# bananaofhappiness/soundscope

Hardware: AMD Instinct MI355X
Metric: audio samples/s analyzed (48 kHz stereo) (higher is better)
Workload: dtype f32 + f64

## Files before the change

soundscope_amd/csrc/ss_batch.cpp:

```cpp
#include "ss_host.h"

using namespace ssh;

namespace {

struct TimingRing {
    static constexpr uint32_t kDepth = 32;
    bool on = false;
    hipEvent_t ev[kDepth * 2 * SS_KERNEL_COUNT] = {};
    uint32_t mask[kDepth] = {};
    uint32_t head = 0, count = 0;
    double ms[SS_KERNEL_COUNT] = {};
    uint64_t launches[SS_KERNEL_COUNT] = {};
    ~TimingRing() { for (auto &e : ev) if (e) (void)hipEventDestroy(e); }
    hipError_t create() { hipError_t r = hipSuccess; for (auto &e : ev) if (r == hipSuccess) r = hipEventCreate(&e); return r; }
    hipError_t mark(int kernel, int edge, hipStream_t stream)
    {
        if (!on) return hipSuccess;
        const int idx = 2 * kernel + edge;
        mask[head] |= 1u << idx;
        return hipEventRecord(ev[(size_t)head * 2 * SS_KERNEL_COUNT + idx], stream);
    }
    void advance() { if (on) { head = (head + 1u) % kDepth; count++; } }
    int collect(hipStream_t stream)
// ... 73 lines not shown
    DevBuf<double> sub, weights, integrated, lra, out2;
    DevBuf<double> seg_state;
    DevBuf<uint64_t> hist, corpus;
    DevBuf<uint32_t> counts;
    DevBuf<unsigned char> raw;
    DevBuf<uint64_t> checks;
    DevBuf<double> series;
    DevBuf<ssk::LoudnessExtremes> extremes;
    Ragged ragged;
    DevBuf<float> render_spec, render_wave;
    DevBuf<uint32_t> col_start;
    uint32_t render_cols = 0, render_wave_cols = 0;
    Columns cols;
    Overlap ov;
    bool corpus_reduced = false;
    int tp_arith = SS_TP_ARITH_F32;
    TimingRing timing;

    uint32_t sub_cap() const { return lay.n_subblocks ? lay.n_subblocks : 1; }
    size_t samples_per_stream() const { return (size_t)cfg.frames_per_stream * cfg.channels; }
};

namespace ssi {
void *batch_corpus_device(ss_batch *b) { return b ? b->corpus.p : nullptr; }
hipStream_t batch_stream(ss_batch *b) { return b ? b->stream : nullptr; }
int batch_device(const ss_batch *b) { return b ? b->device : 0; }
bool &batch_corpus_reduced(ss_batch *b) { return b->corpus_reduced; }
}

namespace {
// ... 310 lines not shown
            L.fft_bytes = rows * b->render_cols * sizeof(float);
        } else {
            L.fft_bytes = rows * L.fft_bin_stride * sizeof(float);
            HIPCHK(b->fft.alloc((size_t)(L.fft_bytes / sizeof(float))));
        }
    }
    if (b->td) {
        HIPCHK(b->state.alloc(cfg->n_streams));
        HIPCHK(b->sub.alloc((size_t)cfg->n_streams * b->sub_cap() * C));
        HIPCHK(b->hist.alloc((size_t)cfg->n_streams * 2 * sst::kHistBins));
        HIPCHK(b->corpus.alloc(2 * sst::kHistBins));
        HIPCHK(b->integrated.alloc(cfg->n_streams));
        HIPCHK(b->lra.alloc(cfg->n_streams));
        HIPCHK(b->counts.alloc((size_t)cfg->n_streams * 2));
        HIPCHK(b->out2.alloc(2));
        std::vector<double> w(C);
        sst::channel_weights(C, w.data());
        HIPCHK(b->weights.upload(w));
        if (cfg->flags & SS_BATCH_LOUDNESS_SERIES) {
            HIPCHK(b->series.alloc((size_t)cfg->n_streams * b->sub_cap() * 2));
            HIPCHK(b->extremes.alloc(cfg->n_streams));
        }
    }
    if (cfg->flags & SS_BATCH_WAVEFORM) {
        if (sh.wave_window > 0xFFFFFFFFull) return SS_ERR_UNSUPPORTED;
        b->wave_window = (uint32_t)sh.wave_window;
        L.n_wave_points = (uint32_t)(2 * sh.wave_bins);
        HIPCHK(b->wave.alloc((size_t)cfg->n_streams * (b->wave_window ? 2 * (size_t)b->wave_window : 2)));
    }

// ... 137 lines not shown
    SS_ON_DEVICE(b);
    if (!b) return SS_ERR_INVALID_ARG;
    HIPCHK(ssk::launch_synth(b->pcm.p, b->cfg.n_streams, b->cfg.frames_per_stream, b->cfg.channels,
                             b->cfg.sample_rate, seed, first_stream_id, b->stream));
    HIPCHK(hipStreamSynchronize(b->stream));
    return SS_OK;
}

int ss_batch_run(ss_batch *b)
{
    SS_ON_DEVICE(b);
    if (!b) return SS_ERR_INVALID_ARG;
    TimingRing &t = b->timing;
    int rc = (t.count >= TimingRing::kDepth || !t.on) ? t.collect(b->stream) : SS_OK;
    if (rc) return rc;
    b->corpus_reduced = false;

    enum class At { first, behind_td, last };
    const bool gain_from_meter = b->cols.on && b->cols.gain_mode == SS_GAIN_REFERENCE;
    const int mode = (t.on || gain_from_meter) ? 0 : b->ov.mode;
    const At at = gain_from_meter ? At::last : mode == 2 ? At::behind_td : At::first;
    auto spectrum_if = [&](At here) { return here == at ? spectrum_step(b, mode != 0) : SS_OK; };

    if ((rc = spectrum_if(At::first))) return rc;

    HIPCHK(t.mark(SS_KERNEL_TIME_DOMAIN, 0, b->stream));
    const ssk::TdParams tdp = b->td ? batch_td_params(b) : ssk::TdParams{};
    if (b->td) {
        HIPCHK(zero_meter(b));
        HIPCHK(t.mark(SS_KERNEL_TIME_DOMAIN, 0, b->stream));
        HIPCHK(ssk::launch_time_domain(tdp, b->stream));
    }
    if ((rc = spectrum_if(At::behind_td))) return rc;
    if (b->td && b->td_plan.fixup) HIPCHK(ssk::launch_time_domain_fixup(tdp, b->stream));
    HIPCHK(t.mark(SS_KERNEL_TIME_DOMAIN, 1, b->stream));

    HIPCHK(t.mark(SS_KERNEL_FINALIZE, 0, b->stream));
    if (b->td) {
        const ssk::FinalizeParams f = batch_gating_params(b);
        HIPCHK(ssk::launch_finalize(f, b->stream));
        if (b->series.p) HIPCHK(ssk::launch_loudness_series(f, b->series.p, b->sub_cap(), b->extremes.p, b->stream));
    }
    HIPCHK(t.mark(SS_KERNEL_FINALIZE, 1, b->stream));

    HIPCHK(t.mark(SS_KERNEL_WAVEFORM, 0, b->stream));
    if ((b->cfg.flags & SS_BATCH_WAVEFORM) && b->wave_window && (!b->wave_fused || b->ragged.on))
        HIPCHK(ssk::launch_waveform(batch_wave_params(b), b->stream));
    HIPCHK(t.mark(SS_KERNEL_WAVEFORM, 1, b->stream));

    if ((rc = spectrum_if(At::last))) return rc;
    if (mode) HIPCHK(b->ov.join(b->stream));
    t.advance();
    return SS_OK;
}

// ... 246 lines not shown
{
    SS_ON_DEVICE(b);
    if (!b || !dst || !b->corpus.p) return SS_ERR_INVALID_ARG;
    return fetch(b, static_cast<uint64_t *>(dst), b->corpus.p, 2 * sst::kHistBins, hipMemcpyDeviceToDevice);
}

int ss_batch_corpus_gate_enqueue(ss_batch *b, ss_comm *comm)
{
    SS_ON_DEVICE(b);
    if (!b) return SS_ERR_INVALID_ARG;
    if (!b->corpus.p) return SS_ERR_INVALID_MODE;
    if (comm) {
        int rc = ss_batch_allreduce_histograms(b, comm, nullptr);
        if (rc) return rc;
    }
    HIPCHK(ssk::launch_hist_eval(b->corpus.p, b->hist_energies, b->hist_bounds, b->out2.p, b->stream));
    return SS_OK;
}

int ss_batch_corpus_gate_read(ss_batch *b, double *integrated, double *lra)
{
    SS_ON_DEVICE(b);
    if (!b) return SS_ERR_INVALID_ARG;
    if (!b->corpus.p) return SS_ERR_INVALID_MODE;
    double r[2];
    int rc = fetch(b, r, b->out2.p, 2);
    if (rc) return rc;
    if (integrated) *integrated = r[0];
    if (lra) *lra = r[1];
    return SS_OK;
// ... 209 lines not shown
```

soundscope_amd/csrc/ss_kernels.h:

```cpp
#pragma once
#include <hip/hip_runtime.h>

#include <mutex>
#include <cstddef>
#include <cstdint>

namespace ssk {

struct DevicePrep {
    std::mutex mu;
    uint64_t done = 0;
};
template <class F>
inline hipError_t prepare_on_device(DevicePrep &p, F &&prepare)
{
    int d = 0;
    if (hipGetDevice(&d) != hipSuccess) d = 0;
    const uint64_t bit = 1ull << (d & 63);
    std::lock_guard<std::mutex> lk(p.mu);
    if (p.done & bit) return hipSuccess;
    const hipError_t e = prepare();
    if (e == hipSuccess) p.done |= bit;
    return e;
}
// ... 115 lines not shown
    uint64_t wave_stride;
    uint32_t wave_window;
    uint32_t halo_frames;
    const uint64_t *frames_of;
    uint32_t tp_f32;
    double *seg_state;
    uint32_t fixup, fix_sub;
    uint32_t split_batch;
    double *st_out;
    double *st_scratch;
    const double *st_weights;
    double st_frames;
    uint32_t st_begin_elem, st_old_total, st_blocks;
};
hipError_t launch_time_domain(const TdParams &p, hipStream_t s, const FftBatchParams *tick_fft = nullptr, bool *tick_fused = nullptr);
hipError_t launch_time_domain_fixup(const TdParams &p, hipStream_t s);
uint32_t td_chunk_frames(uint32_t channels, uint32_t s100);
uint32_t td_split_chunk_frames(uint32_t channels, uint32_t s100);
uint32_t td_resident_waves_per_cu(uint32_t channels, uint32_t s100, uint32_t halo_frames);
uint32_t td_ring_tile_frames(uint32_t channels, uint32_t s100);

struct FinalizeParams {
    const TdConst *k;
    const double *subblocks; uint64_t sub_stride; uint32_t sub_cap;
    const double *hist_energies;
    const double *hist_bounds;
    const double *weights;
    uint64_t *hist;
    uint64_t *corpus_hist;
    uint32_t n_streams, channels;
    uint64_t sub_begin, sub_end;
    double *out_integrated;
    double *out_lra;
    uint32_t *out_counts;
    const uint32_t *sub_end_of;
    const TdState *state;
    double *readings_out;
    const float *readings_peaks_src; float *readings_peaks_dst; uint32_t *readings_flag; uint32_t readings_seq;
};
hipError_t launch_finalize(const FinalizeParams &p, hipStream_t s);
__attribute__((visibility("hidden"))) hipError_t launch_finalize_stream(const FinalizeParams &p, hipStream_t s);
struct LoudnessExtremes { double max_m, max_s; uint32_t at_m, at_s; };
hipError_t launch_loudness_series(const FinalizeParams &p, double *series, uint64_t series_stride, LoudnessExtremes *extremes,
                                  hipStream_t s);
struct ReadingsExtra { const float *peaks_src; float *peaks_dst; uint32_t *flag; uint32_t seq; };
hipError_t launch_hist_eval(const uint64_t *hist2000, const double *energies, const double *bounds,
                            double *out2, hipStream_t s, const ReadingsExtra *peaks = nullptr);
constexpr int kRingScratchDoubles = 320;
constexpr int kRingTickScratch = 264;
constexpr int kRingTickBlocks = 32;
hipError_t launch_ring_energy(const double *ring, uint64_t ring_frames, uint32_t channels,
                              uint64_t end_frame, uint64_t frames, const double *weights,
                              double *out2 ,
                              double *scratch ,
                              hipStream_t s);
// ... 75 lines not shown
```

soundscope_amd/csrc/ss_loudness.hip:

```cpp
#include "ss_kernels.h"

namespace ssk {
__device__ __forceinline__ uint32_t hist_index(const double *__restrict__ bounds, double energy)
{
    const double g = (10.0 * log10(energy) - 0.691 + 70.0) * 10.0;
    int i = g > 0.0 ? (g < (double)(kHistBins - 1) ? (int)g : kHistBins - 1) : 0;
    while (i > 0 && energy < bounds[i]) i--;
    while (i < kHistBins - 1 && energy >= bounds[i + 1]) i++;
    return (uint32_t)i;
}

__device__ __forceinline__ double wave_sum(double v)
{
#pragma unroll
    for (int o = 32; o >= 1; o >>= 1) v += __shfl_xor(v, o, 64);
    return v;
}
__device__ __forceinline__ unsigned long long wave_sum_u64(unsigned long long v)
{
#pragma unroll
    for (int o = 32; o >= 1; o >>= 1) v += __shfl_xor(v, o, 64);
    return v;
}

__device__ __forceinline__ uint32_t first_bad_subblock(const TdState *st, uint32_t C, const double *__restrict__ weights, uint32_t lane)
{
    uint32_t key = 0u;
    if (st) for (uint32_t c = lane; c < C; c += 64u) { const uint32_t k = st->bad_key[c]; if (weights[c] != 0.0 && k > key) key = k; }
#pragma unroll
    for (int o = 32; o >= 1; o >>= 1) { const uint32_t t = (uint32_t)__shfl_xor((int)key, o, 64); key = t > key ? t : key; }
    return ~key;
}

__device__ __forceinline__ void eval_hist(const unsigned long long *hb, const unsigned long long *hs,
                          const double *__restrict__ en, const double *__restrict__ bd,
                          double *out_i, double *out_lra)
{
    const int lane = threadIdx.x & 63;
    double sum = 0.0; unsigned long long cnt = 0;
    for (int i = lane; i < kHistBins; i += 64) { sum += (double)hb[i] * en[i]; cnt += hb[i]; }
    sum = wave_sum(sum); cnt = wave_sum_u64(cnt);
    double integrated;
    if (cnt == 0) integrated = -INFINITY;
    else {
        const double rel = (sum / (double)cnt) * 0.1;
        uint32_t start;
        if (rel < bd[0]) start = 0;
        else { start = hist_index(bd, rel); if (rel > en[start]) start++; }
        double g = 0.0; unsigned long long c2 = 0;
        for (int i = lane; i < kHistBins; i += 64) if ((uint32_t)i >= start) { g += (double)hb[i] * en[i]; c2 += hb[i]; }
        g = wave_sum(g); c2 = wave_sum_u64(c2);
        integrated = c2 ? 10.0 * log10(g / (double)c2) - 0.691 : -INFINITY;
    }
    double power = 0.0; unsigned long long size = 0;
    for (int i = lane; i < kHistBins; i += 64) { power += (double)hs[i] * en[i]; size += hs[i]; }
    power = wave_sum(power); size = wave_sum_u64(size);
    double lra = 0.0;
    if (size != 0) {
        const double integ = 0.01 * (power / (double)size);
        uint32_t index;
        if (integ < bd[0]) index = 0;
        else { index = hist_index(bd, integ); if (integ > en[index]) index++; }
        const int b0 = lane * 16;
        unsigned long long own = 0;
#pragma unroll
        for (int q = 0; q < 16; q++) {
            const int i = b0 + ((q + lane) & 15);
            if (i < kHistBins && (uint32_t)i >= index) own += hs[i];
        }
        unsigned long long incl = own;
#pragma unroll
        for (int o = 1; o < 64; o <<= 1) {
            const unsigned long long t = __shfl_up(incl, o, 64);
            if (lane >= o) incl += t;
        }
        const unsigned long long above = __shfl(incl, 63, 64);
        if (above != 0) {
            const unsigned long long plow = (unsigned long long)((double)(above - 1) * 0.1 + 0.5);
            const unsigned long long phigh = (unsigned long long)((double)(above - 1) * 0.95 + 0.5);
            const unsigned long long excl = incl - own;
            auto energy_of_rank = [&](unsigned long long r) -> double {
                const bool mine = excl <= r && r < incl;
                double e = 0.0;
                if (mine) {
                    unsigned long long acc = excl;
                    int j = b0 > (int)index ? b0 : (int)index;
                    for (;;) { acc += hs[j]; if (acc > r) break; j++; }
                    e = en[j];
                }
                const int src = __ffsll((long long)__ballot(mine)) - 1;
                return __shfl(e, src, 64);
            };
            const double l_en = energy_of_rank(plow), h_en = energy_of_rank(phigh);
            lra = (10.0 * log10(h_en) - 0.691) - (10.0 * log10(l_en) - 0.691);
        }
    }
    if (lane == 0) { if (out_i) *out_i = integrated; if (out_lra) *out_lra = lra; }
}

__device__ __forceinline__ uint32_t ring_back(uint32_t jm, uint32_t q, uint32_t cap)
{
    uint32_t s = jm + cap * 30u - q;
    return s % cap;
}

template <int N, bool DIRECT, int KB = (N < 10 ? N : 10)>
__device__ __forceinline__ double window_energy(const double *__restrict__ P, uint32_t jm, uint32_t cap, uint32_t C,
                                                const double *__restrict__ weights)
{
    constexpr int kBatch = KB;
    static_assert(N % kBatch == 0, "whole batches");
    uint32_t s0 = DIRECT ? jm - (uint32_t)(N - 1) : ring_back(jm, (uint32_t)(N - 1), cap);
    double sum = 0.0;
    for (uint32_t c = 0; c < C; c++) {
        const double w = weights[c];
        if (w == 0.0) continue;
        double cs = 0.0;
        uint32_t sl = s0;
#pragma unroll
        for (int b = 0; b < N; b += kBatch) {
            double v[kBatch];
#pragma unroll
            for (int q = 0; q < kBatch; q++) {
                v[q] = P[(size_t)sl * C + c];
                sl = DIRECT ? sl + 1u : (sl + 1u == cap ? 0u : sl + 1u);
            }
#pragma unroll
            for (int q = 0; q < kBatch; q++) cs += v[q];
        }
        sum += w * cs;
    }
    return sum;
}

template <int N, bool DIRECT>
__device__ __forceinline__ double window_energy_eager(const double *__restrict__ P, uint32_t jm, uint32_t cap, uint32_t C,
                                                      const double *__restrict__ weights)
{
    const uint32_t s0 = DIRECT ? jm - (uint32_t)(N - 1) : ring_back(jm, (uint32_t)(N - 1), cap);
    double sum = 0.0;
    for (uint32_t c = 0; c < C; c += 2) {
        const bool two = c + 1u < C;
        const uint32_t c1 = two ? c + 1u : c;
        const double w0 = weights[c], w1 = weights[c1];
        double v0[N], v1[N];
        uint32_t sl = s0;
#pragma unroll
        for (int q = 0; q < N; q++) {
            v0[q] = P[(size_t)sl * C + c];
            v1[q] = P[(size_t)sl * C + c1];
            sl = DIRECT ? sl + 1u : (sl + 1u == cap ? 0u : sl + 1u);
        }
        double cs0 = 0.0, cs1 = 0.0;
#pragma unroll
        for (int q = 0; q < N; q++) { cs0 += v0[q]; cs1 += v1[q]; }
        if (w0 != 0.0) sum += w0 * cs0;
        if (two && w1 != 0.0) sum += w1 * cs1;
    }
    return sum;
}

template <bool SMALL>
__global__ __launch_bounds__(SMALL ? 256 : 1024) void k_finalize(FinalizeParams p)
{
    __shared__ unsigned long long hb[kHistBins];
    __shared__ unsigned long long hs[kHistBins];
    __shared__ unsigned int counts[2];
    __shared__ uint32_t bad_from_s;
    __shared__ double tab[SMALL ? 2 * kHistBins + 1 : 1];
    const uint32_t stream = blockIdx.x;
    const int lane = threadIdx.x, nthr = (int)blockDim.x;
    unsigned long long *gh = reinterpret_cast<unsigned long long *>(p.hist) + (size_t)stream * 2 * kHistBins;
    unsigned long long *corpus = reinterpret_cast<unsigned long long *>(p.corpus_hist);
    for (int i = lane; i < kHistBins; i += nthr) {
        hb[i] = gh[i]; hs[i] = gh[kHistBins + i];
        if (SMALL) { tab[i] = p.hist_energies[i]; tab[kHistBins + i] = p.hist_bounds[i]; }
    }
    if (SMALL && lane == 0) tab[2 * kHistBins] = p.hist_bounds[kHistBins];
    if (lane < 2) counts[lane] = 0;
    if (lane < 64) {
        const uint32_t bf = first_bad_subblock(p.state ? p.state + stream : nullptr, p.channels, p.weights, (uint32_t)lane);
        if (lane == 0) bad_from_s = bf;
    }
    const double *en = SMALL ? tab : p.hist_energies;
    const double *bd = SMALL ? tab + kHistBins : p.hist_bounds;
    const double bd0 = p.hist_bounds[0];
    const uint64_t sub_end = p.sub_end_of ? p.sub_end_of[stream] : p.sub_end;
    __syncthreads();

    const uint32_t C = p.channels;
    const double S = (double)p.k->s100;
    const double *P = p.subblocks + (size_t)stream * p.sub_stride;
    const uint32_t cap = p.sub_cap;
    const bool direct = p.sub_end <= (uint64_t)cap && p.sub_begin == 0;
    const uint64_t bad_from = bad_from_s;
    uint32_t nb = 0, ns = 0;
    for (uint64_t j = (p.sub_begin > 3 ? p.sub_begin : 3) + lane; j < sub_end; j += nthr) {
        const uint32_t jm = direct ? (uint32_t)j : (uint32_t)(j % cap);
        double sum;
        if (SMALL) sum = direct ? window_energy_eager<4, true>(P, jm, cap, C, p.weights) : window_energy_eager<4, false>(P, jm, cap, C, p.weights);
        else sum = direct ? window_energy<4, true>(P, jm, cap, C, p.weights) : window_energy<4, false>(P, jm, cap, C, p.weights);
        sum /= 4.0 * S;
        nb++;
        if (j > bad_from) sum = __builtin_nan("");
        if (sum >= bd0) atomicAdd(&hb[hist_index(bd, sum)], 1ull);
    }
    if (!p.k->st_off) {
        const uint64_t m_begin = p.sub_begin > 29 ? (p.sub_begin - 29 + 9) / 10 : 0;
        for (uint64_t m = m_begin + lane;; m += nthr) {
            const uint64_t j = 29 + 10 * m;
            if (j >= sub_end) break;
            const uint32_t jm = direct ? (uint32_t)j : (uint32_t)(j % cap);
            double sum;
            if (SMALL) sum = direct ? window_energy_eager<30, true>(P, jm, cap, C, p.weights) : window_energy_eager<30, false>(P, jm, cap, C, p.weights);
            else sum = direct ? window_energy<30, true>(P, jm, cap, C, p.weights) : window_energy<30, false>(P, jm, cap, C, p.weights);
            sum /= 30.0 * S;
            ns++;
            if (j > bad_from) sum = __builtin_nan("");
            if (sum >= bd0) atomicAdd(&hs[hist_index(bd, sum)], 1ull);
        }
    }
    if (nb) atomicAdd(&counts[0], nb);
    if (ns) atomicAdd(&counts[1], ns);
    __syncthreads();
    for (int i = lane; i < kHistBins; i += nthr) {
        const unsigned long long db = hb[i] - gh[i], ds = hs[i] - gh[kHistBins + i];
        if (corpus) {
            if (db) atomicAdd(&corpus[i], db);
            if (ds) atomicAdd(&corpus[kHistBins + i], ds);
        }
        gh[i] = hb[i];
        gh[kHistBins + i] = hs[i];
    }
    if (p.out_counts && lane < 2) p.out_counts[stream * 2 + lane] += counts[lane];
    if (lane < 64)
        eval_hist(hb, hs, en, bd,
                  p.out_integrated ? &p.out_integrated[stream] : nullptr,
                  p.out_lra ? &p.out_lra[stream] : nullptr);
}

__device__ __forceinline__ void gate_stream_range(const double *__restrict__ P, uint32_t cap, uint32_t C, const double *__restrict__ weights,
                                                  const TdConst &K, const double *__restrict__ bd, double bd0, uint64_t sub_begin,
                                                  uint64_t sub_end, uint64_t bad_from, unsigned long long *gh, uint32_t *out_counts,
                                                  uint32_t lane)
{
    const double S = (double)K.s100;
    uint32_t nb = 0, ns = 0;
    for (uint64_t j = (sub_begin > 3 ? sub_begin : 3) + lane; j < sub_end; j += 64) {
        double sum = window_energy_eager<4, false>(P, (uint32_t)(j % cap), cap, C, weights) / (4.0 * S);
        if (j > bad_from) sum = __builtin_nan("");
        nb++;
        if (sum >= bd0) atomicAdd(&gh[hist_index(bd, sum)], 1ull);
    }
    if (!K.st_off) {
        const uint64_t m_begin = sub_begin > 29 ? (sub_begin - 29 + 9) / 10 : 0;
// ... 33 lines not shown
            hb[i] = __hip_atomic_load(&gh[i], __ATOMIC_RELAXED, __HIP_MEMORY_SCOPE_AGENT);
            hs[i] = __hip_atomic_load(&gh[kHistBins + i], __ATOMIC_RELAXED, __HIP_MEMORY_SCOPE_AGENT);
        }
        if (p.readings_peaks_dst) {
            p.readings_peaks_dst[lane] = p.readings_peaks_src[lane];
            p.readings_peaks_dst[64 + lane] = p.readings_peaks_src[64 + lane];
        }
        __syncthreads();
        eval_hist(hb, hs, en, bd, &p.readings_out[0], &p.readings_out[1]);
        if (p.readings_flag) {
            __threadfence_system();
            __syncthreads();
            if (lane == 0) __hip_atomic_store(p.readings_flag, p.readings_seq, __ATOMIC_RELEASE, __HIP_MEMORY_SCOPE_SYSTEM);
        }
    }
}

constexpr uint32_t kFinalizeSmallMax = 64u;
hipError_t launch_finalize(const FinalizeParams &p, hipStream_t s)
{
    if (p.n_streams == 0) return hipSuccess;
    const uint64_t nsub = p.sub_end - p.sub_begin;
    const uint32_t threads = nsub > 2048 ? 1024u : 256u;
    if (p.n_streams <= kFinalizeSmallMax && threads == 256u) hipLaunchKernelGGL(k_finalize<true>, dim3(p.n_streams), dim3(threads), 0, s, p);
    else hipLaunchKernelGGL(k_finalize<false>, dim3(p.n_streams), dim3(threads), 0, s, p);
    return hipGetLastError();
}

hipError_t launch_finalize_stream(const FinalizeParams &p, hipStream_t s)
{
    if (p.n_streams == 0) return hipSuccess;
    hipLaunchKernelGGL(k_finalize_stream, dim3(1), dim3(64), 0, s, p);
    return hipGetLastError();
}

template <int N>
__device__ __forceinline__ double window_energy_head(const double *__restrict__ P, uint32_t j, uint32_t C,
                                                     const double *__restrict__ weights)
{
    double sum = 0.0;
    for (uint32_t c = 0; c < C; c++) {
// ... 333 lines not shown
```

soundscope_amd/csrc/ss_td_body.inc:

```
    using Cfg = TpCfg<FACTOR>;
    constexpr bool kSplitBatch = SPLIT && !RING;
    constexpr bool kSplitCall = SPLIT && RING;
    constexpr bool late = LATE;
    static_assert(!kSplitCall || LATE, "streaming calls hand the state over behind the scan");
    extern __shared__ __attribute__((aligned(16))) unsigned char smem[];
    const uint32_t lane = threadIdx.x & 63u;
    const uint32_t wave_in_block = (uint32_t)__builtin_amdgcn_readfirstlane((int)(threadIdx.x >> 6));
    const uint32_t nwb = SPLIT ? (uint32_t)(blockDim.x >> 6) : (uint32_t)kTdWavesPerBlock;
    const uint32_t gw = SPLIT ? block_id : block_id * kTdWavesPerBlock + wave_in_block;
    const bool fix = p.fixup != 0u;
    const uint32_t wps = fix ? p.nseg - 1u : p.nseg;
    if (gw >= p.n_streams * wps) return;
    const uint32_t stream = gw / wps, sg = gw - stream * wps + (fix ? 1u : 0u);
    TdShare *const sh = reinterpret_cast<TdShare *>(smem + (size_t)nwb * wave_lds_floats * sizeof(float));

    float *tilebuf = reinterpret_cast<float *>(smem) + (size_t)wave_in_block * wave_lds_floats;
    const TdConst &K = *p.k;
    const uint32_t C = CT ? (uint32_t)CT : p.channels;
    const uint32_t S = p.s100;
    const uint32_t nch = 64u / C;
    constexpr bool kRowScan = (CT != 0) && (16 % (CT ? CT : 1) == 0);
    const uint32_t lane_q = (lane & 15u) / C;
    const uint32_t chunk = kRowScan ? (lane >> 4) + 4u * lane_q : lane / C;
    const uint32_t ch = kRowScan ? (lane & 15u) - lane_q * C : lane - chunk * C;
// ... 1205 lines not shown
```

soundscope_amd/csrc/ss_time_domain.hip:

```cpp
#include "ss_td_impl.h"

namespace ssk {
static uint32_t td_lds_blocks(size_t lds)
{
    const uint32_t blocks = (uint32_t)(kTdLdsBytes / lds);
    const uint32_t max_blocks = (4u * kTdWaves) / kTdWavesPerBlock;
    return blocks > max_blocks ? max_blocks : blocks;
}

uint32_t td_chunk_frames(uint32_t C, uint32_t s100)
{
#ifdef SS_TUNING
    if (const char *e = std::getenv("SS_TD_L")) { const int v = std::atoi(e); if (v >= 8 && v <= 128) return (uint32_t)v; }
#endif
    const uint32_t nch = 64u / C;
    const bool rowscan = C == 1 || C == 2 || C == 8;
    static const double occupancy[5] = {8.0, 3.0, 1.6, 1.25, 1.0};
    uint32_t best = 33; double best_cost = 1e300;
    for (uint32_t L : {20u, 25u, 30u, 33u, 35u, 40u, 45u, 49u, 50u, 55u, 60u, 65u}) {
        const TdTile t = td_tile(C, s100, L, kTdHaloFrames, kTdWavesPerBlock, false);
        const uint32_t pieces = t.pieces, tile_len = t.tile_len;
        const uint32_t blocks = td_lds_blocks(t.lds);
        if (blocks == 0) continue;
        const uint32_t rem = tile_len % L;
// ... 49 lines not shown

hipError_t launch_time_domain(const TdParams &p, hipStream_t s, const FftBatchParams *tick_fft, bool *tick_fused)
{
    bool fused_local = false;
    bool *fused = tick_fused ? tick_fused : &fused_local;
    *fused = false;
    if (p.n_streams == 0 || p.n_frames == 0) return hipSuccess;
    const bool ring = p.ring != nullptr;
    switch (p.tp_factor) {
        case 4: return td_launch_f4(p, s, tick_fft, fused, ring);
        case 2: return td_launch_f2(p, s, tick_fft, fused, ring);
        default: return td_launch_f0(p, s, tick_fft, fused, ring);
    }
}

hipError_t launch_time_domain_fixup(const TdParams &p, hipStream_t s)
{
    if (p.n_streams == 0 || p.n_frames == 0 || p.nseg < 2 || !p.seg_state || !p.fix_sub) return hipSuccess;
    TdParams q = p;
    q.fixup = 1u; q.wave_out = nullptr; q.wave_window = 0; q.halo_frames = 0; q.tp_factor = 0;
    bool fused = false;
    return td_launch_f0(q, s, nullptr, &fused, false);
}

}
```

Baseline: 202.2 billion.

## Fuse time-domain fixup, finalize gating and corpus gate into one tail kernel

Replaces the separate fixup launch and finalize launch with a single td_tail kernel. Per-stream groups do the segment fixup, then the last-arriving block per stream (tracked by an atomic arrival counter) runs the gating histogram. A global ticket then lets the final block evaluate the corpus gate in the same kernel, so the later hist_eval launch is skipped when no communicator is used. This removes kernel launches and inter-kernel gaps in exchange for atomic ticketing, extra LDS and more complex synchronization.

```diff
diff --git a/soundscope_amd/csrc/ss_batch.cpp b/soundscope_amd/csrc/ss_batch.cpp
--- a/soundscope_amd/csrc/ss_batch.cpp
+++ b/soundscope_amd/csrc/ss_batch.cpp
@@ -111,6 +111,8 @@
     Columns cols;
     Overlap ov;
     bool corpus_reduced = false;
+    bool corpus_gate_done = false;
+    DevBuf<uint32_t> tail_ticket;
     int tp_arith = SS_TP_ARITH_F32;
     TimingRing timing;
 
@@ -451,6 +453,7 @@
         HIPCHK(b->lra.alloc(cfg->n_streams));
         HIPCHK(b->counts.alloc((size_t)cfg->n_streams * 2));
         HIPCHK(b->out2.alloc(2));
+        HIPCHK(b->tail_ticket.upload(std::vector<uint32_t>((size_t)cfg->n_streams + 1, 0u)));
         std::vector<double> w(C);
         sst::channel_weights(C, w.data());
         HIPCHK(b->weights.upload(w));
@@ -618,7 +621,9 @@
     TimingRing &t = b->timing;
     int rc = (t.count >= TimingRing::kDepth || !t.on) ? t.collect(b->stream) : SS_OK;
     if (rc) return rc;
+    if (t.on) t.mask[t.head] = 0;
     b->corpus_reduced = false;
+    b->corpus_gate_done = false;
 
     enum class At { first, behind_td, last };
     const bool gain_from_meter = b->cols.on && b->cols.gain_mode == SS_GAIN_REFERENCE;
@@ -635,14 +640,14 @@
         HIPCHK(t.mark(SS_KERNEL_TIME_DOMAIN, 0, b->stream));
         HIPCHK(ssk::launch_time_domain(tdp, b->stream));
     }
+    HIPCHK(t.mark(SS_KERNEL_TIME_DOMAIN, 1, b->stream));
     if ((rc = spectrum_if(At::behind_td))) return rc;
-    if (b->td && b->td_plan.fixup) HIPCHK(ssk::launch_time_domain_fixup(tdp, b->stream));
-    HIPCHK(t.mark(SS_KERNEL_TIME_DOMAIN, 1, b->stream));
 
     HIPCHK(t.mark(SS_KERNEL_FINALIZE, 0, b->stream));
     if (b->td) {
         const ssk::FinalizeParams f = batch_gating_params(b);
-        HIPCHK(ssk::launch_finalize(f, b->stream));
+        HIPCHK(ssk::launch_td_tail(tdp, f, b->tail_ticket.p + 1, b->corpus.p ? b->tail_ticket.p : nullptr, b->out2.p, b->stream));
+        b->corpus_gate_done = b->corpus.p != nullptr;
         if (b->series.p) HIPCHK(ssk::launch_loudness_series(f, b->series.p, b->sub_cap(), b->extremes.p, b->stream));
     }
     HIPCHK(t.mark(SS_KERNEL_FINALIZE, 1, b->stream));
@@ -919,6 +924,7 @@
         int rc = ss_batch_allreduce_histograms(b, comm, nullptr);
         if (rc) return rc;
     }
+    if (!comm && b->corpus_gate_done && !b->corpus_reduced) return SS_OK;
     HIPCHK(ssk::launch_hist_eval(b->corpus.p, b->hist_energies, b->hist_bounds, b->out2.p, b->stream));
     return SS_OK;
 }
diff --git a/soundscope_amd/csrc/ss_kernels.h b/soundscope_amd/csrc/ss_kernels.h
--- a/soundscope_amd/csrc/ss_kernels.h
+++ b/soundscope_amd/csrc/ss_kernels.h
@@ -153,7 +153,6 @@
     uint32_t st_begin_elem, st_old_total, st_blocks;
 };
 hipError_t launch_time_domain(const TdParams &p, hipStream_t s, const FftBatchParams *tick_fft = nullptr, bool *tick_fused = nullptr);
-hipError_t launch_time_domain_fixup(const TdParams &p, hipStream_t s);
 uint32_t td_chunk_frames(uint32_t channels, uint32_t s100);
 uint32_t td_split_chunk_frames(uint32_t channels, uint32_t s100);
 uint32_t td_resident_waves_per_cu(uint32_t channels, uint32_t s100, uint32_t halo_frames);
@@ -177,7 +176,7 @@
     double *readings_out;
     const float *readings_peaks_src; float *readings_peaks_dst; uint32_t *readings_flag; uint32_t readings_seq;
 };
-hipError_t launch_finalize(const FinalizeParams &p, hipStream_t s);
+hipError_t launch_td_tail(const TdParams &td, const FinalizeParams &f, uint32_t *arrive, uint32_t *ticket, double *gate_out2, hipStream_t s);
 __attribute__((visibility("hidden"))) hipError_t launch_finalize_stream(const FinalizeParams &p, hipStream_t s);
 struct LoudnessExtremes { double max_m, max_s; uint32_t at_m, at_s; };
 hipError_t launch_loudness_series(const FinalizeParams &p, double *series, uint64_t series_stride, LoudnessExtremes *extremes,
diff --git a/soundscope_amd/csrc/ss_loudness.hip b/soundscope_amd/csrc/ss_loudness.hip
--- a/soundscope_amd/csrc/ss_loudness.hip
+++ b/soundscope_amd/csrc/ss_loudness.hip
@@ -1,244 +1,6 @@
-#include "ss_kernels.h"
+#include "ss_loudness_dev.h"
 
 namespace ssk {
-__device__ __forceinline__ uint32_t hist_index(const double *__restrict__ bounds, double energy)
-{
-    const double g = (10.0 * log10(energy) - 0.691 + 70.0) * 10.0;
-    int i = g > 0.0 ? (g < (double)(kHistBins - 1) ? (int)g : kHistBins - 1) : 0;
-    while (i > 0 && energy < bounds[i]) i--;
-    while (i < kHistBins - 1 && energy >= bounds[i + 1]) i++;
-    return (uint32_t)i;
-}
-
-__device__ __forceinline__ double wave_sum(double v)
-{
-#pragma unroll
-    for (int o = 32; o >= 1; o >>= 1) v += __shfl_xor(v, o, 64);
-    return v;
-}
-__device__ __forceinline__ unsigned long long wave_sum_u64(unsigned long long v)
-{
-#pragma unroll
-    for (int o = 32; o >= 1; o >>= 1) v += __shfl_xor(v, o, 64);
-    return v;
-}
-
-__device__ __forceinline__ uint32_t first_bad_subblock(const TdState *st, uint32_t C, const double *__restrict__ weights, uint32_t lane)
-{
-    uint32_t key = 0u;
-    if (st) for (uint32_t c = lane; c < C; c += 64u) { const uint32_t k = st->bad_key[c]; if (weights[c] != 0.0 && k > key) key = k; }
-#pragma unroll
-    for (int o = 32; o >= 1; o >>= 1) { const uint32_t t = (uint32_t)__shfl_xor((int)key, o, 64); key = t > key ? t : key; }
-    return ~key;
-}
-
-__device__ __forceinline__ void eval_hist(const unsigned long long *hb, const unsigned long long *hs,
-                          const double *__restrict__ en, const double *__restrict__ bd,
-                          double *out_i, double *out_lra)
-{
-    const int lane = threadIdx.x & 63;
-    double sum = 0.0; unsigned long long cnt = 0;
-    for (int i = lane; i < kHistBins; i += 64) { sum += (double)hb[i] * en[i]; cnt += hb[i]; }
-    sum = wave_sum(sum); cnt = wave_sum_u64(cnt);
-    double integrated;
-    if (cnt == 0) integrated = -INFINITY;
-    else {
-        const double rel = (sum / (double)cnt) * 0.1;
-        uint32_t start;
-        if (rel < bd[0]) start = 0;
-        else { start = hist_index(bd, rel); if (rel > en[start]) start++; }
-        double g = 0.0; unsigned long long c2 = 0;
-        for (int i = lane; i < kHistBins; i += 64) if ((uint32_t)i >= start) { g += (double)hb[i] * en[i]; c2 += hb[i]; }
-        g = wave_sum(g); c2 = wave_sum_u64(c2);
-        integrated = c2 ? 10.0 * log10(g / (double)c2) - 0.691 : -INFINITY;
-    }
-    double power = 0.0; unsigned long long size = 0;
-    for (int i = lane; i < kHistBins; i += 64) { power += (double)hs[i] * en[i]; size += hs[i]; }
-    power = wave_sum(power); size = wave_sum_u64(size);
-    double lra = 0.0;
-    if (size != 0) {
-        const double integ = 0.01 * (power / (double)size);
-        uint32_t index;
-        if (integ < bd[0]) index = 0;
-        else { index = hist_index(bd, integ); if (integ > en[index]) index++; }
-        const int b0 = lane * 16;
-        unsigned long long own = 0;
-#pragma unroll
-        for (int q = 0; q < 16; q++) {
-            const int i = b0 + ((q + lane) & 15);
-            if (i < kHistBins && (uint32_t)i >= index) own += hs[i];
-        }
-        unsigned long long incl = own;
-#pragma unroll
-        for (int o = 1; o < 64; o <<= 1) {
-            const unsigned long long t = __shfl_up(incl, o, 64);
-            if (lane >= o) incl += t;
-        }
-        const unsigned long long above = __shfl(incl, 63, 64);
-        if (above != 0) {
-            const unsigned long long plow = (unsigned long long)((double)(above - 1) * 0.1 + 0.5);
-            const unsigned long long phigh = (unsigned long long)((double)(above - 1) * 0.95 + 0.5);
-            const unsigned long long excl = incl - own;
-            auto energy_of_rank = [&](unsigned long long r) -> double {
-                const bool mine = excl <= r && r < incl;
-                double e = 0.0;
-                if (mine) {
-                    unsigned long long acc = excl;
-                    int j = b0 > (int)index ? b0 : (int)index;
-                    for (;;) { acc += hs[j]; if (acc > r) break; j++; }
-                    e = en[j];
-                }
-                const int src = __ffsll((long long)__ballot(mine)) - 1;
-                return __shfl(e, src, 64);
-            };
-            const double l_en = energy_of_rank(plow), h_en = energy_of_rank(phigh);
-            lra = (10.0 * log10(h_en) - 0.691) - (10.0 * log10(l_en) - 0.691);
-        }
-    }
-    if (lane == 0) { if (out_i) *out_i = integrated; if (out_lra) *out_lra = lra; }
-}
-
-__device__ __forceinline__ uint32_t ring_back(uint32_t jm, uint32_t q, uint32_t cap)
-{
-    uint32_t s = jm + cap * 30u - q;
-    return s % cap;
-}
-
-template <int N, bool DIRECT, int KB = (N < 10 ? N : 10)>
-__device__ __forceinline__ double window_energy(const double *__restrict__ P, uint32_t jm, uint32_t cap, uint32_t C,
-                                                const double *__restrict__ weights)
-{
-    constexpr int kBatch = KB;
-    static_assert(N % kBatch == 0, "whole batches");
-    uint32_t s0 = DIRECT ? jm - (uint32_t)(N - 1) : ring_back(jm, (uint32_t)(N - 1), cap);
-    double sum = 0.0;
-    for (uint32_t c = 0; c < C; c++) {
-        const double w = weights[c];
-        if (w == 0.0) continue;
-        double cs = 0.0;
-        uint32_t sl = s0;
-#pragma unroll
-        for (int b = 0; b < N; b += kBatch) {
-            double v[kBatch];
-#pragma unroll
-            for (int q = 0; q < kBatch; q++) {
-                v[q] = P[(size_t)sl * C + c];
-                sl = DIRECT ? sl + 1u : (sl + 1u == cap ? 0u : sl + 1u);
-            }
-#pragma unroll
-            for (int q = 0; q < kBatch; q++) cs += v[q];
-        }
-        sum += w * cs;
-    }
-    return sum;
-}
-
-template <int N, bool DIRECT>
-__device__ __forceinline__ double window_energy_eager(const double *__restrict__ P, uint32_t jm, uint32_t cap, uint32_t C,
-                                                      const double *__restrict__ weights)
-{
-    const uint32_t s0 = DIRECT ? jm - (uint32_t)(N - 1) : ring_back(jm, (uint32_t)(N - 1), cap);
-    double sum = 0.0;
-    for (uint32_t c = 0; c < C; c += 2) {
-        const bool two = c + 1u < C;
-        const uint32_t c1 = two ? c + 1u : c;
-        const double w0 = weights[c], w1 = weights[c1];
-        double v0[N], v1[N];
-        uint32_t sl = s0;
-#pragma unroll
-        for (int q = 0; q < N; q++) {
-            v0[q] = P[(size_t)sl * C + c];
-            v1[q] = P[(size_t)sl * C + c1];
-            sl = DIRECT ? sl + 1u : (sl + 1u == cap ? 0u : sl + 1u);
-        }
-        double cs0 = 0.0, cs1 = 0.0;
-#pragma unroll
-        for (int q = 0; q < N; q++) { cs0 += v0[q]; cs1 += v1[q]; }
-        if (w0 != 0.0) sum += w0 * cs0;
-        if (two && w1 != 0.0) sum += w1 * cs1;
-    }
-    return sum;
-}
-
-template <bool SMALL>
-__global__ __launch_bounds__(SMALL ? 256 : 1024) void k_finalize(FinalizeParams p)
-{
-    __shared__ unsigned long long hb[kHistBins];
-    __shared__ unsigned long long hs[kHistBins];
-    __shared__ unsigned int counts[2];
-    __shared__ uint32_t bad_from_s;
-    __shared__ double tab[SMALL ? 2 * kHistBins + 1 : 1];
-    const uint32_t stream = blockIdx.x;
-    const int lane = threadIdx.x, nthr = (int)blockDim.x;
-    unsigned long long *gh = reinterpret_cast<unsigned long long *>(p.hist) + (size_t)stream * 2 * kHistBins;
-    unsigned long long *corpus = reinterpret_cast<unsigned long long *>(p.corpus_hist);
-    for (int i = lane; i < kHistBins; i += nthr) {
-        hb[i] = gh[i]; hs[i] = gh[kHistBins + i];
-        if (SMALL) { tab[i] = p.hist_energies[i]; tab[kHistBins + i] = p.hist_bounds[i]; }
-    }
-    if (SMALL && lane == 0) tab[2 * kHistBins] = p.hist_bounds[kHistBins];
-    if (lane < 2) counts[lane] = 0;
-    if (lane < 64) {
-        const uint32_t bf = first_bad_subblock(p.state ? p.state + stream : nullptr, p.channels, p.weights, (uint32_t)lane);
-        if (lane == 0) bad_from_s = bf;
-    }
-    const double *en = SMALL ? tab : p.hist_energies;
-    const double *bd = SMALL ? tab + kHistBins : p.hist_bounds;
-    const double bd0 = p.hist_bounds[0];
-    const uint64_t sub_end = p.sub_end_of ? p.sub_end_of[stream] : p.sub_end;
-    __syncthreads();
-
-    const uint32_t C = p.channels;
-    const double S = (double)p.k->s100;
-    const double *P = p.subblocks + (size_t)stream * p.sub_stride;
-    const uint32_t cap = p.sub_cap;
-    const bool direct = p.sub_end <= (uint64_t)cap && p.sub_begin == 0;
-    const uint64_t bad_from = bad_from_s;
-    uint32_t nb = 0, ns = 0;
-    for (uint64_t j = (p.sub_begin > 3 ? p.sub_begin : 3) + lane; j < sub_end; j += nthr) {
-        const uint32_t jm = direct ? (uint32_t)j : (uint32_t)(j % cap);
-        double sum;
-        if (SMALL) sum = direct ? window_energy_eager<4, true>(P, jm, cap, C, p.weights) : window_energy_eager<4, false>(P, jm, cap, C, p.weights);
-        else sum = direct ? window_energy<4, true>(P, jm, cap, C, p.weights) : window_energy<4, false>(P, jm, cap, C, p.weights);
-        sum /= 4.0 * S;
-        nb++;
-        if (j > bad_from) sum = __builtin_nan("");
-        if (sum >= bd0) atomicAdd(&hb[hist_index(bd, sum)], 1ull);
-    }
-    if (!p.k->st_off) {
-        const uint64_t m_begin = p.sub_begin > 29 ? (p.sub_begin - 29 + 9) / 10 : 0;
-        for (uint64_t m = m_begin + lane;; m += nthr) {
-            const uint64_t j = 29 + 10 * m;
-            if (j >= sub_end) break;
-            const uint32_t jm = direct ? (uint32_t)j : (uint32_t)(j % cap);
-            double sum;
-            if (SMALL) sum = direct ? window_energy_eager<30, true>(P, jm, cap, C, p.weights) : window_energy_eager<30, false>(P, jm, cap, C, p.weights);
-            else sum = direct ? window_energy<30, true>(P, jm, cap, C, p.weights) : window_energy<30, false>(P, jm, cap, C, p.weights);
-            sum /= 30.0 * S;
-            ns++;
-            if (j > bad_from) sum = __builtin_nan("");
-            if (sum >= bd0) atomicAdd(&hs[hist_index(bd, sum)], 1ull);
-        }
-    }
-    if (nb) atomicAdd(&counts[0], nb);
-    if (ns) atomicAdd(&counts[1], ns);
-    __syncthreads();
-    for (int i = lane; i < kHistBins; i += nthr) {
-        const unsigned long long db = hb[i] - gh[i], ds = hs[i] - gh[kHistBins + i];
-        if (corpus) {
-            if (db) atomicAdd(&corpus[i], db);
-            if (ds) atomicAdd(&corpus[kHistBins + i], ds);
-        }
-        gh[i] = hb[i];
-        gh[kHistBins + i] = hs[i];
-    }
-    if (p.out_counts && lane < 2) p.out_counts[stream * 2 + lane] += counts[lane];
-    if (lane < 64)
-        eval_hist(hb, hs, en, bd,
-                  p.out_integrated ? &p.out_integrated[stream] : nullptr,
-                  p.out_lra ? &p.out_lra[stream] : nullptr);
-}
-
 __device__ __forceinline__ void gate_stream_range(const double *__restrict__ P, uint32_t cap, uint32_t C, const double *__restrict__ weights,
                                                   const TdConst &K, const double *__restrict__ bd, double bd0, uint64_t sub_begin,
                                                   uint64_t sub_end, uint64_t bad_from, unsigned long long *gh, uint32_t *out_counts,
@@ -302,17 +64,6 @@
             if (lane == 0) __hip_atomic_store(p.readings_flag, p.readings_seq, __ATOMIC_RELEASE, __HIP_MEMORY_SCOPE_SYSTEM);
         }
     }
-}
-
-constexpr uint32_t kFinalizeSmallMax = 64u;
-hipError_t launch_finalize(const FinalizeParams &p, hipStream_t s)
-{
-    if (p.n_streams == 0) return hipSuccess;
-    const uint64_t nsub = p.sub_end - p.sub_begin;
-    const uint32_t threads = nsub > 2048 ? 1024u : 256u;
-    if (p.n_streams <= kFinalizeSmallMax && threads == 256u) hipLaunchKernelGGL(k_finalize<true>, dim3(p.n_streams), dim3(threads), 0, s, p);
-    else hipLaunchKernelGGL(k_finalize<false>, dim3(p.n_streams), dim3(threads), 0, s, p);
-    return hipGetLastError();
 }
 
 hipError_t launch_finalize_stream(const FinalizeParams &p, hipStream_t s)
diff --git a/soundscope_amd/csrc/ss_loudness_dev.h b/soundscope_amd/csrc/ss_loudness_dev.h
--- /dev/null
+++ b/soundscope_amd/csrc/ss_loudness_dev.h
@@ -0,0 +1,276 @@
+#pragma once
+#include "ss_kernels.h"
+
+namespace ssk {
+__device__ __forceinline__ uint32_t hist_index(const double *__restrict__ bounds, double energy)
+{
+    const double g = (10.0 * log10(energy) - 0.691 + 70.0) * 10.0;
+    int i = g > 0.0 ? (g < (double)(kHistBins - 1) ? (int)g : kHistBins - 1) : 0;
+    while (i > 0 && energy < bounds[i]) i--;
+    while (i < kHistBins - 1 && energy >= bounds[i + 1]) i++;
+    return (uint32_t)i;
+}
+
+__device__ __forceinline__ double wave_sum(double v)
+{
+#pragma unroll
+    for (int o = 32; o >= 1; o >>= 1) v += __shfl_xor(v, o, 64);
+    return v;
+}
+__device__ __forceinline__ unsigned long long wave_sum_u64(unsigned long long v)
+{
+#pragma unroll
+    for (int o = 32; o >= 1; o >>= 1) v += __shfl_xor(v, o, 64);
+    return v;
+}
+
+__device__ __forceinline__ uint32_t first_bad_subblock(const TdState *st, uint32_t C, const double *__restrict__ weights, uint32_t lane)
+{
+    uint32_t key = 0u;
+    if (st) for (uint32_t c = lane; c < C; c += 64u) { const uint32_t k = st->bad_key[c]; if (weights[c] != 0.0 && k > key) key = k; }
+#pragma unroll
+    for (int o = 32; o >= 1; o >>= 1) { const uint32_t t = (uint32_t)__shfl_xor((int)key, o, 64); key = t > key ? t : key; }
+    return ~key;
+}
+
+__device__ __forceinline__ void eval_hist(const unsigned long long *hb, const unsigned long long *hs,
+                          const double *__restrict__ en, const double *__restrict__ bd,
+                          double *out_i, double *out_lra)
+{
+    const int lane = threadIdx.x & 63;
+    double sum = 0.0; unsigned long long cnt = 0;
+    for (int i = lane; i < kHistBins; i += 64) { sum += (double)hb[i] * en[i]; cnt += hb[i]; }
+    sum = wave_sum(sum); cnt = wave_sum_u64(cnt);
+    double integrated;
+    if (cnt == 0) integrated = -INFINITY;
+    else {
+        const double rel = (sum / (double)cnt) * 0.1;
+        uint32_t start;
+        if (rel < bd[0]) start = 0;
+        else { start = hist_index(bd, rel); if (rel > en[start]) start++; }
+        double g = 0.0; unsigned long long c2 = 0;
+        for (int i = lane; i < kHistBins; i += 64) if ((uint32_t)i >= start) { g += (double)hb[i] * en[i]; c2 += hb[i]; }
+        g = wave_sum(g); c2 = wave_sum_u64(c2);
+        integrated = c2 ? 10.0 * log10(g / (double)c2) - 0.691 : -INFINITY;
+    }
+    double power = 0.0; unsigned long long size = 0;
+    for (int i = lane; i < kHistBins; i += 64) { power += (double)hs[i] * en[i]; size += hs[i]; }
+    power = wave_sum(power); size = wave_sum_u64(size);
+    double lra = 0.0;
+    if (size != 0) {
+        const double integ = 0.01 * (power / (double)size);
+        uint32_t index;
+        if (integ < bd[0]) index = 0;
+        else { index = hist_index(bd, integ); if (integ > en[index]) index++; }
+        const int b0 = lane * 16;
+        unsigned long long own = 0;
+#pragma unroll
+        for (int q = 0; q < 16; q++) {
+            const int i = b0 + ((q + lane) & 15);
+            if (i < kHistBins && (uint32_t)i >= index) own += hs[i];
+        }
+        unsigned long long incl = own;
+#pragma unroll
+        for (int o = 1; o < 64; o <<= 1) {
+            const unsigned long long t = __shfl_up(incl, o, 64);
+            if (lane >= o) incl += t;
+        }
+        const unsigned long long above = __shfl(incl, 63, 64);
+        if (above != 0) {
+            const unsigned long long plow = (unsigned long long)((double)(above - 1) * 0.1 + 0.5);
+            const unsigned long long phigh = (unsigned long long)((double)(above - 1) * 0.95 + 0.5);
+            const unsigned long long excl = incl - own;
+            auto energy_of_rank = [&](unsigned long long r) -> double {
+                const bool mine = excl <= r && r < incl;
+                double e = 0.0;
+                if (mine) {
+                    unsigned long long acc = excl;
+                    int j = b0 > (int)index ? b0 : (int)index;
+                    for (;;) { acc += hs[j]; if (acc > r) break; j++; }
+                    e = en[j];
+                }
+                const int src = __ffsll((long long)__ballot(mine)) - 1;
+                return __shfl(e, src, 64);
+            };
+            const double l_en = energy_of_rank(plow), h_en = energy_of_rank(phigh);
+            lra = (10.0 * log10(h_en) - 0.691) - (10.0 * log10(l_en) - 0.691);
+        }
+    }
+    if (lane == 0) { if (out_i) *out_i = integrated; if (out_lra) *out_lra = lra; }
+}
+
+__device__ __forceinline__ uint32_t ring_back(uint32_t jm, uint32_t q, uint32_t cap)
+{
+    uint32_t s = jm + cap * 30u - q;
+    return s % cap;
+}
+
+template <int N, bool DIRECT, int KB = (N < 10 ? N : 10)>
+__device__ __forceinline__ double window_energy(const double *__restrict__ P, uint32_t jm, uint32_t cap, uint32_t C,
+                                                const double *__restrict__ weights)
+{
+    constexpr int kBatch = KB;
+    static_assert(N % kBatch == 0, "whole batches");
+    uint32_t s0 = DIRECT ? jm - (uint32_t)(N - 1) : ring_back(jm, (uint32_t)(N - 1), cap);
+    double sum = 0.0;
+    for (uint32_t c = 0; c < C; c++) {
+        const double w = weights[c];
+        if (w == 0.0) continue;
+        double cs = 0.0;
+        uint32_t sl = s0;
+#pragma unroll
+        for (int b = 0; b < N; b += kBatch) {
+            double v[kBatch];
+#pragma unroll
+            for (int q = 0; q < kBatch; q++) {
+                v[q] = P[(size_t)sl * C + c];
+                sl = DIRECT ? sl + 1u : (sl + 1u == cap ? 0u : sl + 1u);
+            }
+#pragma unroll
+            for (int q = 0; q < kBatch; q++) cs += v[q];
+        }
+        sum += w * cs;
+    }
+    return sum;
+}
+
+template <int N, bool DIRECT>
+__device__ __forceinline__ double window_energy_eager(const double *__restrict__ P, uint32_t jm, uint32_t cap, uint32_t C,
+                                                      const double *__restrict__ weights)
+{
+    const uint32_t s0 = DIRECT ? jm - (uint32_t)(N - 1) : ring_back(jm, (uint32_t)(N - 1), cap);
+    double sum = 0.0;
+    for (uint32_t c = 0; c < C; c += 2) {
+        const bool two = c + 1u < C;
+        const uint32_t c1 = two ? c + 1u : c;
+        const double w0 = weights[c], w1 = weights[c1];
+        double v0[N], v1[N];
+        uint32_t sl = s0;
+#pragma unroll
+        for (int q = 0; q < N; q++) {
+            v0[q] = P[(size_t)sl * C + c];
+            v1[q] = P[(size_t)sl * C + c1];
+            sl = DIRECT ? sl + 1u : (sl + 1u == cap ? 0u : sl + 1u);
+        }
+        double cs0 = 0.0, cs1 = 0.0;
+#pragma unroll
+        for (int q = 0; q < N; q++) { cs0 += v0[q]; cs1 += v1[q]; }
+        if (w0 != 0.0) sum += w0 * cs0;
+        if (two && w1 != 0.0) sum += w1 * cs1;
+    }
+    return sum;
+}
+
+constexpr uint32_t kFinalizeSmallMax = 64u;
+
+struct GateLds {
+    unsigned long long *hb, *hs;
+    double *tab;
+    unsigned int *counts;
+    uint32_t *bad_from;
+    uint32_t *last;
+};
+constexpr size_t kGateLdsBytes = (2 * kHistBins + 2 * kHistBins + 1) * 8 + 4 * 4;
+__device__ __forceinline__ GateLds gate_lds(unsigned char *smem)
+{
+    GateLds l;
+    l.hb = reinterpret_cast<unsigned long long *>(smem);
+    l.hs = l.hb + kHistBins;
+    l.tab = reinterpret_cast<double *>(l.hs + kHistBins);
+    l.counts = reinterpret_cast<unsigned int *>(l.tab + 2 * kHistBins + 1);
+    l.bad_from = l.counts + 2;
+    l.last = l.counts + 3;
+    return l;
+}
+
+template <bool SMALL>
+__device__ __forceinline__ void gate_batch_stream(const FinalizeParams &p, const uint32_t stream, const GateLds &l)
+{
+    unsigned long long *const hb = l.hb, *const hs = l.hs;
+    unsigned int *const counts = l.counts;
+    double *const tab = l.tab;
+    const int lane = threadIdx.x, nthr = (int)blockDim.x;
+    unsigned long long *gh = reinterpret_cast<unsigned long long *>(p.hist) + (size_t)stream * 2 * kHistBins;
+    unsigned long long *corpus = reinterpret_cast<unsigned long long *>(p.corpus_hist);
+    for (int i = lane; i < kHistBins; i += nthr) {
+        hb[i] = gh[i]; hs[i] = gh[kHistBins + i];
+        if (SMALL) { tab[i] = p.hist_energies[i]; tab[kHistBins + i] = p.hist_bounds[i]; }
+    }
+    if (SMALL && lane == 0) tab[2 * kHistBins] = p.hist_bounds[kHistBins];
+    if (lane < 2) counts[lane] = 0;
+    if (lane < 64) {
+        const uint32_t bf = first_bad_subblock(p.state ? p.state + stream : nullptr, p.channels, p.weights, (uint32_t)lane);
+        if (lane == 0) *l.bad_from = bf;
+    }
+    const double *en = SMALL ? tab : p.hist_energies;
+    const double *bd = SMALL ? tab + kHistBins : p.hist_bounds;
+    const double bd0 = p.hist_bounds[0];
+    const uint64_t sub_end = p.sub_end_of ? p.sub_end_of[stream] : p.sub_end;
+    __syncthreads();
+
+    const uint32_t C = p.channels;
+    const double S = (double)p.k->s100;
+    const double *P = p.subblocks + (size_t)stream * p.sub_stride;
+    const uint32_t cap = p.sub_cap;
+    const bool direct = p.sub_end <= (uint64_t)cap && p.sub_begin == 0;
+    const uint64_t bad_from = *l.bad_from;
+    uint32_t nb = 0, ns = 0;
+    for (uint64_t j = (p.sub_begin > 3 ? p.sub_begin : 3) + lane; j < sub_end; j += nthr) {
+        const uint32_t jm = direct ? (uint32_t)j : (uint32_t)(j % cap);
+        double sum;
+        if (SMALL) sum = direct ? window_energy_eager<4, true>(P, jm, cap, C, p.weights) : window_energy_eager<4, false>(P, jm, cap, C, p.weights);
+        else sum = direct ? window_energy<4, true>(P, jm, cap, C, p.weights) : window_energy<4, false>(P, jm, cap, C, p.weights);
+        sum /= 4.0 * S;
+        nb++;
+        if (j > bad_from) sum = __builtin_nan("");
+        if (sum >= bd0) atomicAdd(&hb[hist_index(bd, sum)], 1ull);
+    }
+    if (!p.k->st_off) {
+        const uint64_t m_begin = p.sub_begin > 29 ? (p.sub_begin - 29 + 9) / 10 : 0;
+        for (uint64_t m = m_begin + lane;; m += nthr) {
+            const uint64_t j = 29 + 10 * m;
+            if (j >= sub_end) break;
+            const uint32_t jm = direct ? (uint32_t)j : (uint32_t)(j % cap);
+            double sum;
+            if (SMALL) sum = direct ? window_energy_eager<30, true>(P, jm, cap, C, p.weights) : window_energy_eager<30, false>(P, jm, cap, C, p.weights);
+            else sum = direct ? window_energy<30, true>(P, jm, cap, C, p.weights) : window_energy<30, false>(P, jm, cap, C, p.weights);
+            sum /= 30.0 * S;
+            ns++;
+            if (j > bad_from) sum = __builtin_nan("");
+            if (sum >= bd0) atomicAdd(&hs[hist_index(bd, sum)], 1ull);
+        }
+    }
+    if (nb) atomicAdd(&counts[0], nb);
+    if (ns) atomicAdd(&counts[1], ns);
+    __syncthreads();
+    for (int i = lane; i < kHistBins; i += nthr) {
+        const unsigned long long db = hb[i] - gh[i], ds = hs[i] - gh[kHistBins + i];
+        if (corpus) {
+            if (db) atomicAdd(&corpus[i], db);
+            if (ds) atomicAdd(&corpus[kHistBins + i], ds);
+        }
+        gh[i] = hb[i];
+        gh[kHistBins + i] = hs[i];
+    }
+    if (p.out_counts && lane < 2) p.out_counts[stream * 2 + lane] += counts[lane];
+    if (lane < 64)
+        eval_hist(hb, hs, en, bd,
+                  p.out_integrated ? &p.out_integrated[stream] : nullptr,
+                  p.out_lra ? &p.out_lra[stream] : nullptr);
+}
+
+template <bool TABLES_READY>
+__device__ __forceinline__ void corpus_gate_eval(const FinalizeParams &p, double *out2, const GateLds &l)
+{
+    const unsigned long long *corpus = reinterpret_cast<const unsigned long long *>(p.corpus_hist);
+    for (int i = threadIdx.x; i < kHistBins; i += (int)blockDim.x) {
+        l.hb[i] = __hip_atomic_load(&corpus[i], __ATOMIC_RELAXED, __HIP_MEMORY_SCOPE_AGENT);
+        l.hs[i] = __hip_atomic_load(&corpus[kHistBins + i], __ATOMIC_RELAXED, __HIP_MEMORY_SCOPE_AGENT);
+        if (!TABLES_READY) { l.tab[i] = p.hist_energies[i]; l.tab[kHistBins + i] = p.hist_bounds[i]; }
+    }
+    if (!TABLES_READY && threadIdx.x == 0) l.tab[2 * kHistBins] = p.hist_bounds[kHistBins];
+    __syncthreads();
+    if (threadIdx.x < 64) eval_hist(l.hb, l.hs, l.tab, l.tab + kHistBins, &out2[0], &out2[1]);
+}
+
+}
diff --git a/soundscope_amd/csrc/ss_td_body.inc b/soundscope_amd/csrc/ss_td_body.inc
--- a/soundscope_amd/csrc/ss_td_body.inc
+++ b/soundscope_amd/csrc/ss_td_body.inc
@@ -7,7 +7,11 @@
     const uint32_t lane = threadIdx.x & 63u;
     const uint32_t wave_in_block = (uint32_t)__builtin_amdgcn_readfirstlane((int)(threadIdx.x >> 6));
     const uint32_t nwb = SPLIT ? (uint32_t)(blockDim.x >> 6) : (uint32_t)kTdWavesPerBlock;
+#ifdef SS_TD_BODY_UNIT
+    const uint32_t gw = (SS_TD_BODY_UNIT);
+#else
     const uint32_t gw = SPLIT ? block_id : block_id * kTdWavesPerBlock + wave_in_block;
+#endif
     const bool fix = p.fixup != 0u;
     const uint32_t wps = fix ? p.nseg - 1u : p.nseg;
     if (gw >= p.n_streams * wps) return;
diff --git a/soundscope_amd/csrc/ss_td_tail.hip b/soundscope_amd/csrc/ss_td_tail.hip
--- /dev/null
+++ b/soundscope_amd/csrc/ss_td_tail.hip
@@ -0,0 +1,125 @@
+#include "ss_td_impl.h"
+#include "ss_loudness_dev.h"
+
+namespace ssk {
+
+struct TdTailParams {
+    TdParams td;
+    FinalizeParams fin;
+    uint32_t fix_waves;
+    uint32_t groups;
+    uint32_t *arrive;
+    uint32_t L, tile_len, wave_floats;
+    uint32_t *ticket;
+    double *gate_out2;
+};
+
+template <int CT>
+__device__ __forceinline__ void td_fix_unit(const TdParams &p, const uint32_t L, const uint32_t tile_len, const uint32_t wave_lds_floats,
+                                            const uint32_t unit)
+{
+    constexpr int FACTOR = 0, WAVE = 0, WPS = 4;
+    constexpr bool RING = false, SPLIT = false, LATE = false;
+    const uint32_t halo_frames = (uint32_t)kTdHaloFrames;
+    constexpr int kTdPrefetch = 7;
+#define SS_TD_BODY_UNIT unit
+#include "ss_td_body.inc"
+#undef SS_TD_BODY_UNIT
+}
+
+template <int CT, bool SMALL, int THREADS>
+__global__ __launch_bounds__(THREADS, THREADS == 256 && !SMALL ? 4 : 1) void k_td_tail(TdTailParams q)
+{
+    extern __shared__ __attribute__((aligned(16))) unsigned char smem[];
+    const uint32_t stream = CT >= 0 ? blockIdx.x / q.groups : blockIdx.x;
+    const GateLds l = gate_lds(smem);
+    if constexpr (CT >= 0) {
+        const uint32_t wave = (uint32_t)__builtin_amdgcn_readfirstlane((int)(threadIdx.x >> 6));
+        const uint32_t per = q.td.nseg - 1u;
+        const uint32_t k = (blockIdx.x - stream * q.groups) * q.fix_waves + wave;
+        if (wave < q.fix_waves && k < per) td_fix_unit<CT>(q.td, q.L, q.tile_len, q.wave_floats, stream * per + k);
+        if (q.groups > 1u) {
+            __threadfence();
+            __syncthreads();
+            if (threadIdx.x == 0) {
+                const bool last = __hip_atomic_fetch_add(&q.arrive[stream], 1u, __ATOMIC_RELAXED, __HIP_MEMORY_SCOPE_AGENT) == q.groups - 1u;
+                if (last) __hip_atomic_store(&q.arrive[stream], 0u, __ATOMIC_RELAXED, __HIP_MEMORY_SCOPE_AGENT);
+                *l.last = last ? 1u : 0u;
+            }
+            __syncthreads();
+            if (!*l.last) return;
+            __threadfence();
+        } else {
+            __syncthreads();
+        }
+    }
+    gate_batch_stream<SMALL>(q.fin, stream, l);
+    if (!q.ticket) return;
+    __builtin_amdgcn_s_waitcnt(0);
+    __syncthreads();
+    if (threadIdx.x == 0)
+        *l.last = __hip_atomic_fetch_add(q.ticket, 1u, __ATOMIC_RELAXED, __HIP_MEMORY_SCOPE_AGENT) == q.fin.n_streams - 1u ? 1u : 0u;
+    __syncthreads();
+    if (!*l.last) return;
+    corpus_gate_eval<SMALL>(q.fin, q.gate_out2, l);
+    if (threadIdx.x == 0) __hip_atomic_store(q.ticket, 0u, __ATOMIC_RELAXED, __HIP_MEMORY_SCOPE_AGENT);
+}
+
+template <int CT, bool SMALL, int THREADS>
+static hipError_t td_tail_launch(const TdTailParams &q, size_t lds, hipStream_t s)
+{
+    auto fn = k_td_tail<CT, SMALL, THREADS>;
+    static DevicePrep prepared;
+    const hipError_t pe = prepare_on_device(prepared, [fn] {
+        return hipFuncSetAttribute(reinterpret_cast<const void *>(fn), hipFuncAttributeMaxDynamicSharedMemorySize, (int)kTdLdsBytes);
+    });
+    if (pe != hipSuccess) return pe;
+    hipLaunchKernelGGL(fn, dim3(q.fin.n_streams * (CT >= 0 ? q.groups : 1u)), dim3(THREADS), lds, s, q);
+    return hipGetLastError();
+}
+
+template <int CT>
+static hipError_t td_tail_launch_c(const TdTailParams &q, size_t lds, uint32_t threads, bool small, hipStream_t s)
+{
+    constexpr bool kFix = CT >= 0;
+    if (threads > 256u) return td_tail_launch<CT, false, kFix ? 512 : 1024>(q, lds, s);
+    return small ? td_tail_launch<CT, true, 256>(q, lds, s) : td_tail_launch<CT, false, 256>(q, lds, s);
+}
+
+hipError_t launch_td_tail(const TdParams &p, const FinalizeParams &f, uint32_t *arrive, uint32_t *ticket, double *gate_out2, hipStream_t s)
+{
+    if (f.n_streams == 0) return hipSuccess;
+    if (p.n_streams != f.n_streams || (ticket && (!f.corpus_hist || !gate_out2))) return hipErrorInvalidValue;
+    TdTailParams q{};
+    q.td = p; q.fin = f; q.ticket = ticket; q.gate_out2 = gate_out2; q.arrive = arrive; q.groups = 1;
+    const bool fix = p.n_frames != 0 && p.nseg >= 2 && p.seg_state && p.fix_sub;
+    const uint64_t nsub = f.sub_end - f.sub_begin;
+    const bool long_streams = nsub > 2048;
+    const bool small = f.n_streams <= kFinalizeSmallMax && !long_streams && !(fix && p.nseg - 1u > 4u);
+    const uint32_t threads = long_streams ? (fix ? 512u : 1024u) : 256u;
+    size_t lds = kGateLdsBytes;
+    if (fix) {
+        if (p.split_batch != kTdSplitNone) return hipErrorInvalidValue;
+        q.td.fixup = 1u; q.td.wave_out = nullptr; q.td.wave_window = 0; q.td.halo_frames = 0; q.td.tp_factor = 0;
+        const uint32_t C = p.channels, S = p.s100;
+        q.L = td_chunk_frames(C, S);
+        const TdTile t = td_tile(C, S, q.L, (uint32_t)kTdHaloFrames, 1u, false);
+        q.tile_len = t.tile_len; q.wave_floats = t.wave_floats;
+        const size_t wave_bytes = (size_t)t.wave_floats * sizeof(float);
+        const uint32_t per = p.nseg - 1u;
+        uint32_t waves = threads / 64u;
+        if (waves > per) waves = per;
+        if ((size_t)waves * wave_bytes > kTdLdsBytes) waves = (uint32_t)(kTdLdsBytes / wave_bytes);
+        if (waves == 0) return hipErrorInvalidValue;
+        q.fix_waves = waves;
+        q.groups = (per + waves - 1u) / waves;
+        if ((q.groups > 1u && !arrive) || (uint64_t)f.n_streams * q.groups > 0x7FFFFFFFull) return hipErrorInvalidValue;
+        if ((size_t)waves * wave_bytes > lds) lds = (size_t)waves * wave_bytes;
+        if (p.channels == 8) return td_tail_launch_c<8>(q, lds, threads, small, s);
+        if (p.channels == 2) return td_tail_launch_c<2>(q, lds, threads, small, s);
+        return td_tail_launch_c<0>(q, lds, threads, small, s);
+    }
+    return td_tail_launch_c<-1>(q, lds, threads, small, s);
+}
+
+}
diff --git a/soundscope_amd/csrc/ss_time_domain.hip b/soundscope_amd/csrc/ss_time_domain.hip
--- a/soundscope_amd/csrc/ss_time_domain.hip
+++ b/soundscope_amd/csrc/ss_time_domain.hip
@@ -87,13 +87,4 @@
     }
 }
 
-hipError_t launch_time_domain_fixup(const TdParams &p, hipStream_t s)
-{
-    if (p.n_streams == 0 || p.n_frames == 0 || p.nseg < 2 || !p.seg_state || !p.fix_sub) return hipSuccess;
-    TdParams q = p;
-    q.fixup = 1u; q.wave_out = nullptr; q.wave_window = 0; q.halo_frames = 0; q.tp_factor = 0;
-    bool fused = false;
-    return td_launch_f0(q, s, nullptr, &fused, false);
 }
-
-}
```

After: 201.9 billion. About the same (-0.2%).
